# yifita/DSS

Hardware: AMD Instinct MI355X
Metric: Msplats/s fwd+bwd @512^2 (higher is better)
Workload: dtype f32; 1 GPU; BASELINE configs[1]: bunny-8000 x4 jitter = 32684 pts/cloud, 1 camera(s), 512x512, K=5, fwd+bwd (setup+raster+blend and their backward), grad_out=randn(seed 1), variance scale h precomputed (kNN-7 outside the step; see value_with_knn); points_per_cloud=32684, cameras=1, image_size=512, points_per_pixel=5, h_precomputed=True, parallelism=rows1, launch=eager, steps_per_graph_launch=1, full=False

## Files before the change

dss_amd/_lib.py:

```python
import ctypes
import os
import threading

import torch

_HERE = os.path.dirname(os.path.abspath(__file__))
LIB_PATH = os.environ.get("DSS_HIP_LIBRARY") or os.path.join(_HERE, "csrc", "libdss_hip.so")

_lib = None
_lock = threading.Lock()

_c_int, _c_i64, _c_f32, _c_vp, _c_sz = (ctypes.c_int, ctypes.c_int64, ctypes.c_float,
                                         ctypes.c_void_p, ctypes.c_size_t)

SIGNATURES = {
    "dss_version": (_c_int, []),
    "dss_last_error": (ctypes.c_char_p, []),
    "dss_band_rows": (_c_int, [_c_int, _c_int, _c_int]),
    "dss_set_option": (_c_int, [_c_int, _c_int]),
    "dss_get_option": (_c_int, [_c_int]),
    "dss_splat_forward_workspace": (_c_sz, [_c_int, _c_i64, _c_int, _c_int, _c_int]),
    "dss_splat_forward_clean_bytes": (_c_sz, [_c_int, _c_i64, _c_int]),
    "dss_splat_forward": (_c_int, [_c_vp] * 6 + [_c_int, _c_i64, _c_f32, _c_int, _c_int, _c_int, _c_int, _c_int]
                          + [_c_vp] * 5 + [_c_vp, _c_sz, _c_vp]),
# ... 77 lines not shown
    "dss_camera_backward": (_c_int, [_c_vp] * 5 + [_c_int, _c_i64, _c_int, _c_vp, _c_vp, _c_f32, _c_vp, _c_vp, _c_vp, _c_sz, _c_vp]),
    "dss_phong_backward_camera": (_c_int, [_c_vp] * 6 + [_c_int, _c_i64, _c_int] + [_c_vp] * 4 + [_c_int, _c_int, _c_vp, _c_f32,
                                                                                                 _c_vp, _c_vp, _c_sz, _c_vp]),
    "dss_phong_backward_lights_workspace": (_c_sz, [_c_int, _c_i64, _c_int]),
    "dss_phong_backward_lights": (_c_int, [_c_vp] * 6 + [_c_int, _c_i64, _c_int] + [_c_vp] * 4 + [_c_int, _c_int, _c_vp, _c_f32]
                                  + [_c_vp] * 4 + [_c_vp, _c_sz, _c_vp]),
    "dss_blend_backward": (_c_int, [_c_vp] * 10 + [_c_int, _c_i64, _c_int, _c_int, _c_int, _c_int, _c_int, _c_vp, _c_vp]),
    "dss_blend_backward_scatter": (_c_int, [_c_vp] * 4 + [_c_int] * 5 + [_c_i64, _c_vp, _c_vp]),
}


def load():
    global _lib
    if _lib is not None:
        return _lib
    with _lock:
        if _lib is None:
            if not os.path.exists(LIB_PATH):
                raise RuntimeError(
                    "dss_amd: %s not found. Build it with `make -C dss_amd/csrc` (or "
                    "`python -c 'import __graft_entry__ as g; g.build()'`). There is no CPU fallback."
                    % LIB_PATH)
            lib = ctypes.CDLL(LIB_PATH)
            for name, (res, args) in SIGNATURES.items():
                fn = getattr(lib, name)
                fn.restype = res
                fn.argtypes = args
            _lib = lib
    return _lib


WS_ORDER_SAVE, WS_ORDER_REUSE = 0x10, 0x20
WS_BAND_OUTPUTS = 0x40
OPT_LEAN_WORKSPACE, OPT_BACKWARD_TPW, OPT_BACKWARD_ADDR64, OPT_BACKWARD_FUSED, OPT_KNN_QUERY = 0, 1, 2, 3, 4


def set_option(option: int, value: int) -> int:
    lib = load()
    old = lib.dss_get_option(option)
    check(lib.dss_set_option(option, value), "dss_set_option")
    return old


def check(rc: int, what: str) -> None:
    if rc != 0:
        msg = load().dss_last_error().decode("utf-8", "replace")
        raise RuntimeError("%s failed (%d): %s" % (what, rc, msg))


def ptr(t):
    return None if t is None else ctypes.c_void_p(t.data_ptr())


def stream_ptr(device):
    return ctypes.c_void_p(torch.cuda.current_stream(device).cuda_stream)


def require_gpu(t: torch.Tensor, name: str, dtype=None) -> torch.Tensor:
    if not isinstance(t, torch.Tensor):
        raise TypeError("%s must be a torch.Tensor" % name)
    if not t.is_cuda:
        raise RuntimeError("dss_amd: %s is on %s; the HIP path needs GPU tensors (no CPU fallback)"
                           % (name, t.device))
    if dtype is not None and t.dtype != dtype:
        raise RuntimeError("dss_amd: %s must be %s, got %s" % (name, dtype, t.dtype))
    return t.contiguous()

# ... 50 lines not shown
```

dss_amd/csrc/api.hip:

```cpp
#include <stdarg.h>
#include <atomic>
#include "common.h"

namespace dss {

static thread_local char g_err[512] = "";

void set_error(const char *fmt, ...)
{
    va_list ap;
    va_start(ap, fmt);
    vsnprintf(g_err, sizeof(g_err), fmt, ap);
    va_end(ap);
}

int check_launch(const char *what)
{
    const hipError_t e = hipGetLastError();
    if (e != hipSuccess) {
        set_error("%s: %s", what, hipGetErrorString(e));
        return DSS_ERR_LAUNCH;
    }
    return DSS_OK;
}
// ... 21 lines not shown
    }
    return cus;
}

unsigned resident_blocks(int dev, const void *kernel, int block)
{
    DeviceCache *dc = (dev >= 0 && dev < DSS_MAX_DEVICES) ? &g_dev[dev] : nullptr;
    int i = 0;
    for (; dc && i < DSS_MAX_RESIDENT; ++i) {
        const void *k = dc->kernel[i].load(std::memory_order_acquire);
        if (k == nullptr) break;
        const unsigned long long v = dc->value[i].load(std::memory_order_acquire);
        if (k == kernel && (v >> 32) == (unsigned)block) return (unsigned)v;
    }
    int per_cu = 0;
    (void)hipOccupancyMaxActiveBlocksPerMultiprocessor(&per_cu, kernel, block, 0);
    (void)hipGetLastError();
    if (per_cu < 1) per_cu = 1;
    const void *expect = nullptr;
    if (dc && i < DSS_MAX_RESIDENT && dc->kernel[i].compare_exchange_strong(expect, kernel, std::memory_order_acq_rel))
        dc->value[i].store((unsigned long long)block << 32 | (unsigned)per_cu, std::memory_order_release);
    return (unsigned)per_cu;
}

}

extern "C" int dss_set_option(int option, int value)
{
    if (option < 0 || option >= DSS_OPT_COUNT) { dss::set_error("dss_set_option: unknown option %d", option); return DSS_ERR_INVALID_ARGUMENT; }
    if (option == DSS_OPT_BACKWARD_TPW && !(value == 0 || value == 1 || value == 2 || value == 4)) {
        dss::set_error("dss_set_option: DSS_OPT_BACKWARD_TPW takes 0 (automatic), 1, 2 or 4");
        return DSS_ERR_INVALID_ARGUMENT;
    }
    dss::g_opt[option].store(value, std::memory_order_relaxed);
    return DSS_OK;
}
extern "C" int dss_get_option(int option) { return dss::option(option); }

extern "C" int dss_band_rows(int row0, int row1, int row_cycle)
{
    if (row1 <= row0) return 0;
    if (row_cycle <= 1) return row1 - row0;
    const int span = row1 - row0, period = 8 * row_cycle;
    const int full = span / period, rem = span - full * period;
    return full * 8 + (rem < 8 ? rem : 8);
}

extern "C" int dss_version(void) { return DSS_HIP_VERSION; }
extern "C" const char *dss_last_error(void) { return dss::g_err; }
```

dss_amd/csrc/raster_backward.hip:

```cpp
#include <stdlib.h>
#include <type_traits>
#include "point_bodies.h"

namespace dss {

__device__ __forceinline__ uint32_t float_key(float f)
{
    const uint32_t b = __float_as_uint(f);
    return (b & 0x80000000u) ? ~b : (b | 0x80000000u);
}
__device__ __forceinline__ float key_float(uint32_t k)
{
    const uint32_t b = (k & 0x80000000u) ? (k & 0x7fffffffu) : ~k;
    return __uint_as_float(b);
}

#define MED_THREADS 256
#define MED_BINS 2048
#define MED_PTS_PER_WG 2048

__device__ __forceinline__ void select_bin(const uint32_t *hist, uint32_t k, bool k_is_lower_median,
                                           uint32_t *s_scan , uint32_t &bin_out, uint32_t &k_out,
                                           uint32_t &total_out)
{
// ... 885 lines not shown
{
    v = row_sum16(v);
    if (RP == 1) return v;
    const float a = __int_as_float(__builtin_amdgcn_readlane(__float_as_int(v), 0));
    const float b = __int_as_float(__builtin_amdgcn_readlane(__float_as_int(v), 16));
    const float c = __int_as_float(__builtin_amdgcn_readlane(__float_as_int(v), 32));
    const float d = __int_as_float(__builtin_amdgcn_readlane(__float_as_int(v), 48));
    if (RP == 4) return (a + b) + (c + d);
    return grp == 0 ? a + b : c + d;
}
template <int TPW>
__device__ __forceinline__ int tasks_max(int v)
{
    int m = __builtin_amdgcn_readlane(v, 0);
    if (TPW >= 2) m = max(m, __builtin_amdgcn_readlane(v, 32));
    if (TPW >= 4) m = max(m, max(__builtin_amdgcn_readlane(v, 16), __builtin_amdgcn_readlane(v, 48)));
    return m;
}


extern "C" __device__ unsigned long long dss_dispatch_id(void) __asm("llvm.amdgcn.dispatch.id");

#define DSS_BACKWARD_FUSED_DEFAULT 4
#define FB_THREADS 256
#define FB_BUCKETS 256
#define FB_CAND_MAX 4096
#define FB_HIST 1024
#define FB_TAG_RS 0
#define FB_TAGS (8 * 64)
#define FB_SPIN_LIMIT (1 << 20)
#define FB_ALPHA_PER_WG 2048
#define FB_MAX_SEG 256
#define FB_MEDIAN_LDS (FB_CAND_MAX + FB_HIST + 3 * FB_MAX_SEG + 32)
#define FB_KEY_LO 0xB7800000u
#define FB_KEY_HI 0xBF800000u
__device__ __forceinline__ uint32_t fb_bucket(uint32_t key)
{
    const uint32_t c = min(max(key, FB_KEY_LO), FB_KEY_HI - 1u);
    return (c - FB_KEY_LO) >> 19;
}

struct FusedPrep {
    const uint8_t *visible;
    uint32_t *seg_count;
    int32_t *vis_list;
    uint32_t *keys;
    uint32_t *chunk_hist;
    uint2 *seg_range;
    unsigned long long *tags;
    float *rs;
    int64_t P;
    int chunks, per;
    float radii_s;
};

__device__ __forceinline__ unsigned long long fb_launch_tag()
{
    const unsigned long long q = (unsigned long long)__builtin_amdgcn_queue_ptr();
    return dss_dispatch_id() * 0x9E3779B97F4A7C15ull ^ (q << 17) ^ (q >> 7) ^ 0x5851F42D4C957F2Dull;
}

__device__ __forceinline__ uint32_t fb_block_excl_scan(uint32_t v, uint32_t *s_w , uint32_t &total)
{
    const int lane = threadIdx.x & 63, wid = threadIdx.x >> 6;
    const uint32_t x = wave_incl_scan(v);
    __syncthreads();
    if (lane == 63) s_w[wid] = x;
    __syncthreads();
    uint32_t woff = 0;
    total = 0;
#pragma unroll
    for (int w = 0; w < FB_THREADS / 64; ++w) {
        const uint32_t c = s_w[w];
        if (w < wid) woff += c;
        total += c;
    }
    return woff + x - v;
}

template <int PER>
__device__ __forceinline__ void fb_prep_segment(const FusedPrep &F, int c, const float *__restrict__ radii,
                                                const int64_t *__restrict__ first_idx, const int64_t *__restrict__ num_pts,
// ... 297 lines not shown
            if (__ballot(!ok) == 0ull) break;
            __builtin_amdgcn_s_sleep(8);
        }
    }
    __syncthreads();
}

template <int PER>
__global__ __launch_bounds__(FB_THREADS) void fb_prep_kernel(const FusedPrep F, const float *__restrict__ radii,
                                                             const int64_t *__restrict__ first_idx,
                                                             const int64_t *__restrict__ num_pts, int N,
                                                             float *__restrict__ grad_pts, float *__restrict__ grad_feat, int C,
                                                             const float *__restrict__ grad_out, float *__restrict__ alpha_plane,
                                                             size_t npix)
{
    if ((int)blockIdx.x >= F.chunks) {
        const size_t i0 = (size_t)(blockIdx.x - F.chunks) * FB_ALPHA_PER_WG + threadIdx.x;
        if (C == 3) {
            const float4 *g4 = reinterpret_cast<const float4 *>(grad_out);
            float a[FB_ALPHA_PER_WG / FB_THREADS];
#pragma unroll
            for (int u = 0; u < FB_ALPHA_PER_WG / FB_THREADS; ++u) a[u] = g4[min(i0 + (size_t)u * FB_THREADS, npix - 1)].w;
#pragma unroll
            for (int u = 0; u < FB_ALPHA_PER_WG / FB_THREADS; ++u)
                if (i0 + (size_t)u * FB_THREADS < npix) alpha_plane[i0 + (size_t)u * FB_THREADS] = a[u];
        } else {
            for (int u = 0; u < FB_ALPHA_PER_WG / FB_THREADS; ++u) {
                const size_t i = i0 + (size_t)u * FB_THREADS;
                if (i < npix) alpha_plane[i] = grad_out[i * (C + 1) + C];
            }
        }
        return;
    }
    __shared__ uint32_t s_fb[2 * FB_BUCKETS + 160];
    fb_prep_segment<PER>(F, (int)blockIdx.x, radii, first_idx, num_pts, N, grad_pts, grad_feat, C, s_fb);
}
__global__ __launch_bounds__(FB_THREADS) void fb_median_kernel(const FusedPrep F, const int64_t *__restrict__ first_idx,
                                                               const int64_t *__restrict__ num_pts)
{
    __shared__ uint32_t s_fb[FB_MEDIAN_LDS];
    const float v = fb_median(F, (int)blockIdx.x, first_idx, num_pts, s_fb);
    if (threadIdx.x == 0) F.rs[blockIdx.x] = v;
}

#ifndef DSS_BAND_RB
#define DSS_BAND_RB 8
#endif
#define BAND_SHARE 512
template <int C, bool SEG, int TPW, bool A32, bool CYC = false, bool PREP = false, bool BAND = false>
__global__ __launch_bounds__(256) void render_backward_kernel(
    const float *__restrict__ grad_out, const float *__restrict__ grad_alpha ,
    const int32_t *__restrict__ idx, const float *__restrict__ qv,
    const float *__restrict__ wsum, const float *__restrict__ scaler, const float *__restrict__ points,
    const float *__restrict__ radii, const float *__restrict__ rs, const int64_t *__restrict__ first_idx,
    const int64_t *__restrict__ num_pts, const uint32_t *__restrict__ vis_count,
    const int32_t *__restrict__ vis_list, int n_seg, int seg_pts, int N, int S, int K, int Crt, float clip, int row0,
    int rows, uint32_t large_waves, float *__restrict__ grad_feat, float *__restrict__ grad_pts, int tshift = 3,
    const float *__restrict__ world = nullptr ,
    const float *__restrict__ Mproj = nullptr ,
    const FusedPrep F = FusedPrep() ,
    int astride = 1 ,
    const OwnArgs OW = OwnArgs{nullptr, 1} )
{
    constexpr int CM = (C > 0) ? C : BLEND_MAX_C;
    constexpr int KF = 8;
    constexpr int GS = 64 / TPW;
// ... 53 lines not shown
        return chunked ? ((t / max(CH, 1u)) * 8u + xcd) * CH + (t % max(CH, 1u)) : t;
    };
    const uint32_t wave_u = (uint32_t)__builtin_amdgcn_readfirstlane((int)qof(t0));
    if (!PREP && !BAND && wave_u >= n_groups) return;
    const bool has_tasks = wave < n_waves && wave_u < n_groups;
    const uint32_t t_first = (uint32_t)__builtin_amdgcn_readfirstlane((int)t0);

    auto task_ids = [&](uint32_t q) -> int {
        int off[TPW];
#pragma unroll
        for (int g = 0; g < TPW; ++g) {
            const uint32_t t = (uint32_t)TPW * q + (uint32_t)g;
            off[g] = -1;
            if (t < count) {
                if (SEG) {
                    const int seg = (int)__popcll(__ballot(seg_excl <= t)) - 1;
                    const uint32_t excl = (uint32_t)__builtin_amdgcn_readlane((int)seg_excl, seg);
                    off[g] = seg * seg_pts + (int)(t - excl);
                } else {
                    off[g] = (int)t;
                }
            }
        }
        int o = off[0];
#pragma unroll
        for (int g = 1; g < TPW; ++g) o = (grp == g) ? off[g] : o;
        return o >= 0 ? vis_list[o] : -1;
    };
    const NdcMap ndc(S);
    const size_t plane = (size_t)rows * S;
    __shared__ uint32_t s_deal[2];
    const uint32_t blk4 = (blockIdx.x - first_block) * 4u;
    auto dyn_group = [&](uint32_t i) -> uint32_t { return blk4 + (i & 3u) + (i >> 2) * n_waves; };
    float *s_rec = reinterpret_cast<float *>(s_pool);
    int32_t *s_band = reinterpret_cast<int32_t *>(s_pool) + (BAND ? 7 * BAND_SHARE : 0);
    __shared__ uint32_t s_bcnt[2];
    __shared__ float s_brs[BAND ? 64 : 1];
    constexpr int BAND_NSH = 24;
    int32_t b_id[2] = {-1, -1};
    int b_n[2] = {-1, -1};
    float b_py[2] = {0.f, 0.f}, b_ry[2] = {0.f, 0.f};
    if (BAND) {
        if (threadIdx.x == 0) { s_bcnt[0] = 0; s_bcnt[1] = 0; }
        __syncthreads();
        const uint32_t n_wg = gridDim.x - first_block, wg = blockIdx.x - first_block;
#pragma unroll
        for (int j = 0; j < 2; ++j) {
            const uint32_t e = wg + ((uint32_t)threadIdx.x + 256u * (uint32_t)j) * n_wg;
            if (e < count) {
                int sg = 0;
#pragma unroll
                for (int st = FB_MAX_SEG / 2; st >= 1; st >>= 1) sg += (sg + st < FB_MAX_SEG && s_bseg[sg + st] <= e) ? st : 0;
                b_id[j] = vis_list[(size_t)sg * seg_pts + (e - s_bseg[sg])];
            }
        }
#pragma unroll
        for (int j = 0; j < 2; ++j) {
            if (b_id[j] >= 0) {
                const size_t i = (size_t)b_id[j];
                const int slot = (int)threadIdx.x + 256 * j;
                const float px_ = points[3 * i], py_ = points[3 * i + 1], pz_ = points[3 * i + 2];
                const float2 rr_ = reinterpret_cast<const float2 *>(radii)[i];
                const float sc_ = scaler ? scaler[i] : 0.0f;
                b_py[j] = py_;
                b_ry[j] = rr_.y;
                b_n[j] = find_cloud(b_id[j], first_idx, num_pts, N);
// ... 29 lines not shown
                }
            }
            const unsigned long long m = __ballot(keep);
            uint32_t base = 0;
            if (lane == 0 && m) base = atomicAdd(&s_bcnt[WHICH], (uint32_t)__popcll(m));
            base = (uint32_t)__builtin_amdgcn_readfirstlane((int)base);
            if (keep) {
                s_band[WHICH * BAND_SHARE + base + __builtin_amdgcn_mbcnt_hi((unsigned)(m >> 32), __builtin_amdgcn_mbcnt_lo((unsigned)m, 0u))] =
                    (int)threadIdx.x + 256 * j;
            } else if (b_id[j] >= 0) {
                const size_t i = (size_t)b_id[j];
                if (WHICH == 0) {
                    if (grad_feat)
                        for (int ch = 0; ch < Cn; ++ch) grad_feat[i * Cn + ch] = 0.0f;
                } else {
                    grad_pts[3 * i] = 0.0f; grad_pts[3 * i + 1] = 0.0f; grad_pts[3 * i + 2] = 0.0f;
                }
            }
        }
        __syncthreads();
    };
    const uint32_t wave_in_wg = threadIdx.x >> 6;
    auto band_ids = [&](uint32_t q, int which) -> int {
        const uint32_t t = (uint32_t)TPW * q + (uint32_t)grp;
        return t < s_bcnt[which] ? s_band[which * BAND_SHARE + t] : -1;
    };
    if (PREP || BAND) {
        if (threadIdx.x < 2) s_deal[threadIdx.x] = 4u;
        __syncthreads();
    }
    auto run_tasks = [&](auto phase_tag) {
    constexpr int PH = decltype(phase_tag)::value;
    uint32_t t_cur = t_first;
    const uint32_t b_groups = BAND ? (s_bcnt[PH == 2 ? 1 : 0] + TPW - 1u) / TPW : 0u;
    int p_nx = BAND ? band_ids(wave_in_wg, PH == 2 ? 1 : 0) : task_ids(wave_u);
    for (;;) {
        const int b_slot = BAND ? max(p_nx, 0) : 0;
        const int b_word = (BAND && p_nx >= 0) ? reinterpret_cast<const int32_t *>(s_rec)[b_slot] : -1;
        const int p = BAND ? (b_word >= 0 ? (b_word & ((1 << BAND_NSH) - 1)) : -1) : p_nx;
        const int p_cloud = b_word >= 0 ? (b_word >> BAND_NSH) : -1;
        uint32_t t_next, q_next;
        if (BAND) {
            uint32_t i_next = 0;
            if (lane == 0) i_next = atomicAdd(&s_deal[PH == 2 ? 1 : 0], 1u);
            q_next = t_next = (uint32_t)__builtin_amdgcn_readfirstlane((int)i_next);
        } else if (PREP) {
            uint32_t i_next = 0;
            if (lane == 0) i_next = atomicAdd(&s_deal[PH == 2 ? 1 : 0], 1u);
            q_next = t_next = dyn_group((uint32_t)__builtin_amdgcn_readfirstlane((int)i_next));
        } else {
            t_next = t_cur + t_stride;
            q_next = qof(t_next);
        }
        const bool more = q_next < (BAND ? b_groups : n_groups);
        if (more) p_nx = BAND ? band_ids(q_next, PH == 2 ? 1 : 0) : task_ids(q_next);
        float px = 0.f, py = 0.f, pz = -1.f, rx = 0.f, ry = 0.f, sc = 0.f, cur_r = 0.f;
        float wx = 0.f, wy = 0.f, wz = 0.f;
        int n = -1;
        if (BAND) {
            if (p >= 0) {
                px = s_rec[BAND_SHARE + b_slot]; py = s_rec[2 * BAND_SHARE + b_slot]; pz = s_rec[3 * BAND_SHARE + b_slot];
                rx = s_rec[4 * BAND_SHARE + b_slot]; ry = s_rec[5 * BAND_SHARE + b_slot]; sc = s_rec[6 * BAND_SHARE + b_slot];
                n = p_cloud;
                if (PH != 1) cur_r = s_brs[n];
            }
        } else if (p >= 0) {
            px = points[3 * (size_t)p]; py = points[3 * (size_t)p + 1]; pz = points[3 * (size_t)p + 2];
            const float2 rr = reinterpret_cast<const float2 *>(radii)[p];
            rx = rr.x; ry = rr.y;
            sc = scaler ? scaler[p] : 0.0f;
            if (world) { wx = world[3 * (size_t)p]; wy = world[3 * (size_t)p + 1]; wz = world[3 * (size_t)p + 2]; }
            for (int cld = 0; cld < N; ++cld) {
                const int64_t f = first_idx[cld];
                const bool own = (int64_t)p >= f && (int64_t)p < f + num_pts[cld];
                n = own ? cld : n;
                if (PH != 1) cur_r = own ? (PREP ? __hip_atomic_load(&rs[cld], __ATOMIC_RELAXED, __HIP_MEMORY_SCOPE_AGENT) : rs[cld]) : cur_r;
            }
        }
        const int nn = max(n, 0);
        typedef float f2 __attribute__((ext_vector_type(2)));
        f2 gx2 = {0.0f, 0.0f}, gy2 = {0.0f, 0.0f};
        if constexpr (PH != 1) {
// ... 227 lines not shown
#pragma unroll
                    for (int k = 0; k < KF; ++k) {
                        vi[k] = -1; qk[k] = 0.0f;
                        if (k < K) { vi[k] = pi[k]; qk[k] = pq[k]; }
                    }
                    cum = wsum[pix];
#pragma unroll
                    for (int ch = 0; ch < CM; ++ch) gch[ch] = (ch < Cn) ? go[ch] : 0.0f;
#pragma unroll
                    for (int k = 0; k < KF; ++k) {
                        const bool hit = (k < K) && vi[k] == (int32_t)p;
                        q_sel = hit ? qk[k] : q_sel;
                        found = found || hit;
                    }
                } else {
                    cum = 0.0f;
                    for (int k = 0; k < K; ++k) {
                        const int32_t v = pi[k];
                        if (v == (int32_t)p) { found = true; q_sel = pq[k]; }
                        if (!wsum && v >= 0) cum += ewa_weight(pq[k], scaler[v]);
                    }
                    if (wsum) cum = wsum[pix];
                    else if (cum < 1e-4f) cum = 1e-4f;
#pragma unroll
                    for (int ch = 0; ch < CM; ++ch) gch[ch] = (ch < Cn) ? go[ch] : 0.0f;
                }
                if (!found) continue;
                const float wn = ewa_weight(q_sel, sc) * fast_rcp(cum);
#pragma unroll
                for (int ch = 0; ch < CM; ++ch)
                    if (ch < Cn) acc[ch] = fmaf(gch[ch], wn, acc[ch]);
            }
        }
        if (PH != 1) {
            gx = task_sum<RP>(gx, grp);
            gy = task_sum<RP>(gy, grp);
        }
        if (PH != 2) {
#pragma unroll
            for (int ch = 0; ch < CM; ++ch)
                if (ch < Cn) acc[ch] = task_sum<RP>(acc[ch], grp);
        }
        if (PH == 1) {
            if (l == 0 && rp == 0 && p >= 0 && n >= 0 && grad_feat) {
#pragma unroll
                for (int ch = 0; ch < CM; ++ch)
                    if (ch < Cn) grad_feat[(size_t)p * Cn + ch] = acc[ch];
            }
        } else if (l == 0 && rp == 0 && p >= 0 && n >= 0) {
            if (clip > 0.0f) {
                const float nrm = sqrtf(gx * gx + gy * gy);
                const float k = fminf(nrm, clip) * fast_rcp(fmaxf(nrm, 1e-12f));
                gx *= k;
                gy *= k;
            }
            float o0 = gx, o1 = gy, o2 = 0.0f;
            if (world) {
                const float *m = Mproj + 16 * nn;
                const float cx = wx * m[0] + wy * m[4] + wz * m[8] + m[12];
                const float cy = wx * m[1] + wy * m[5] + wz * m[9] + m[13];
                const float w = wx * m[3] + wy * m[7] + wz * m[11] + m[15];
                const float iw = 1.0f / w;
                const float nx = cx * iw, ny = cy * iw;
                float t3[3];
#pragma unroll
                for (int i = 0; i < 3; ++i) {
                    const float jx = (m[i * 4 + 0] - nx * m[i * 4 + 3]) * iw;
                    const float jy = (m[i * 4 + 1] - ny * m[i * 4 + 3]) * iw;
                    t3[i] = jx * gx + jy * gy + 0.0f;
                }
                o0 = t3[0]; o1 = t3[1]; o2 = t3[2];
            }
            grad_pts[3 * (size_t)p] = o0;
            grad_pts[3 * (size_t)p + 1] = o1;
            grad_pts[3 * (size_t)p + 2] = o2;
            if (PH == 0 && grad_feat) {
#pragma unroll
                for (int ch = 0; ch < CM; ++ch)
                    if (ch < Cn) grad_feat[(size_t)p * Cn + ch] = acc[ch];
            }
        }
        if (!more) break;
        t_cur = t_next;
    }
    };
    if (BAND) {
        PREP_MARK(0);
        if (grad_feat) {
            band_filter(std::integral_constant<int, 0>{});
            PREP_MARK(8);
            if (wave_in_wg * TPW < s_bcnt[0]) run_tasks(std::integral_constant<int, 1>{});
        }
        PREP_MARK(1);
        if (PREP) fb_wait_rs(F, N, fb_launch_tag());
        if ((int)threadIdx.x < N)
            s_brs[threadIdx.x] = PREP ? __hip_atomic_load(&rs[threadIdx.x], __ATOMIC_RELAXED, __HIP_MEMORY_SCOPE_AGENT) : rs[threadIdx.x];
        __syncthreads();
        PREP_MARK(2);
        band_filter(std::integral_constant<int, 1>{});
        PREP_MARK(9);
        if (wave_in_wg * TPW < s_bcnt[1]) run_tasks(std::integral_constant<int, 2>{});
        PREP_MARK(3);
    } else if (!PREP) {
        run_tasks(std::integral_constant<int, 0>{});
    } else {
        PREP_MARK(0);
        if (has_tasks) run_tasks(std::integral_constant<int, 1>{});
        PREP_MARK(1);
        fb_wait_rs(F, N, fb_launch_tag());
        PREP_MARK(2);
        if (has_tasks) run_tasks(std::integral_constant<int, 2>{});
        PREP_MARK(3);
    }
// ... 2 lines not shown
__global__ __launch_bounds__(256) void zbuf_backward_kernel(const int32_t *__restrict__ idx,
                                                            const float *__restrict__ grad_zbuf,
                                                            size_t npix, int K, float *__restrict__ grad_pts)
{
    const size_t i = (size_t)blockIdx.x * blockDim.x + threadIdx.x;
    if (i >= npix) return;
    for (int k = 0; k < K; ++k) {
        const float g = grad_zbuf[i * K + k];
        if (g == 0.0f) continue;
        const int32_t p = idx[i * K + k];
        if (p < 0) break;
        atomicAdd(&grad_pts[3 * (size_t)p + 2], g);
    }
}

__global__ __launch_bounds__(256) void clip_grad_kernel(float *__restrict__ grad, int64_t P, float clip)
{
    const int64_t p = (int64_t)blockIdx.x * blockDim.x + threadIdx.x;
    if (p >= P) return;
    const float gx = grad[3 * p], gy = grad[3 * p + 1], gz = grad[3 * p + 2];
    const float nrm = sqrtf(gx * gx + gy * gy + gz * gz);
    const float scaler = fminf(nrm, clip);
    const float den = fmaxf(nrm, 1e-12f);
    grad[3 * p] = gx / den * scaler;
    grad[3 * p + 1] = gy / den * scaler;
    grad[3 * p + 2] = gz / den * scaler;
}

}

using namespace dss;

struct PrepLayout {
    size_t seg_count, vis_list, vis_keys, chunk_hist, seg_range, rs, alpha, tags, bytes;
    int chunks, per;
    int f_chunks, f_per;
};
static PrepLayout prep_layout(int N, int64_t P, int S, bool band = false)
{
    PrepLayout L;
    const size_t n = N > 0 ? N : 1, p = P > 0 ? (size_t)P : 1;
    L.per = prep_points_per_thread(P);
    const size_t seg = (size_t)L.per * PREP_THREADS;
    L.chunks = (int)((p + seg - 1) / seg);
    L.f_per = 1;
    const size_t f_max_seg = (band && p > (size_t)2 * FB_THREADS * PREP_MAX_SEG) ? FB_MAX_SEG : PREP_MAX_SEG;
    while (L.f_per < 16 && (size_t)L.f_per * FB_THREADS * f_max_seg < p) L.f_per *= 2;
    L.f_chunks = (int)((p + (size_t)L.f_per * FB_THREADS - 1) / ((size_t)L.f_per * FB_THREADS));
    size_t off = 0;
    L.seg_count = off;  off += (size_t)FB_MAX_SEG * 4;
    L.vis_list = off;   off += align_up(p * 4, 256);
    L.vis_keys = off;   off += align_up(p * 8, 256);
    L.chunk_hist = off; off += align_up(n * (size_t)FB_MAX_SEG * 256 * 4, 256);
    L.seg_range = off;  off += align_up(n * (size_t)FB_MAX_SEG * 8, 256);
    L.tags = off;       off += align_up((size_t)FB_TAGS * 8, 256);
    L.rs = off;         off += align_up(n * 4, 256);
    L.alpha = off;      off += align_up(n * (size_t)(S > 0 ? S : 0) * (size_t)(S > 0 ? S : 0) * 4, 256);
    L.bytes = off;
    return L;
}

struct LongLayout {
    size_t hist, vis_count, vis_list, rs, alpha, cell_of, sorted, cell_start, cell_total, block_hist, bytes;
};
static LongLayout long_layout(int N, int64_t P, int S)
{
    LongLayout L;
    const size_t n = N > 0 ? N : 1, s = S > 0 ? S : 1, p = P > 0 ? (size_t)P : 1;
    const size_t cells = (size_t)make_cells(N > 0 ? N : 1, S > 0 ? S : 1).total;
    size_t off = 0;
    L.hist = off;       L.vis_count = off + 3 * n * MED_BINS * 4;
    off += align_up(3 * n * MED_BINS * 4 + 256, 256);
    L.vis_list = off;   off += align_up(p * 4, 256);
    L.rs = off;         off += align_up(n * 4, 256);
    L.alpha = off;      off += align_up(n * s * s * 4, 256);
    L.cell_of = off;    off += align_up(p * 4, 256);
    L.sorted = off;     off += align_up(p * 4, 256);
    L.cell_start = off; off += align_up(cells * 4, 256);
    L.cell_total = off; off += align_up(cells * 4, 256);
    L.block_hist = off; off += align_up(cell_blocks(P) * cells * 4, 256);
    L.bytes = off;
    return L;
}

static const decltype(&backward_compact_kernel<2>) compact_by_per[] = {backward_compact_kernel<2>, backward_compact_kernel<4>};
static const decltype(&band_filter_kernel<2>) band_filter_by_per[] = {band_filter_kernel<2>, band_filter_kernel<4>};
static const decltype(&fb_prep_kernel<1>) fb_prep_by_per[] = {fb_prep_kernel<1>, fb_prep_kernel<2>, fb_prep_kernel<4>,
                                                              fb_prep_kernel<8>, fb_prep_kernel<16>};
// ... 223 lines not shown
        }
    }
    const int rows = dss_band_rows(row0, row1, row_cycle);
    int tshift = 3;
    for (int c = row_cycle; c > 1; c >>= 1) ++tshift;
    const bool cyc = row_cycle > 1;
    if (P == 0) return DSS_OK;
    if (P > 0x7ffffff0ll) { set_error("dss_render_backward: P too large"); return DSS_ERR_UNSUPPORTED; }
    OwnArgs OW = {(grad_full != nullptr && (rows < S || cyc)) ? grad_full + C : nullptr, C + 1};
    const bool own_given = occ_full != nullptr && (rows < S || cyc);
    if (own_given) { OW.alpha = occ_full; OW.astride = 1; }
    const int own = OW.alpha != nullptr ? 1 : 0;
    if (!grad_out || !points || !radii || !visible || !first_idx || !num_pts || !grad_pts ||
        (grad_feat && (!idx || !qvalue || !scaler))) {
        set_error("dss_render_backward: NULL tensor pointer");
        return DSS_ERR_INVALID_ARGUMENT;
    }
    const size_t need = dss_render_backward_workspace(N, P, S);
    if (!workspace || workspace_bytes < need) {
        set_error("dss_render_backward: workspace %zu bytes < required %zu", workspace_bytes, need);
        return DSS_ERR_WORKSPACE;
    }
    if (((uintptr_t)grad_out & 15u) && C == 3) { set_error("dss_render_backward: grad_out must be 16-byte aligned"); return DSS_ERR_INVALID_ARGUMENT; }

    hipStream_t st = as_stream(stream);
    char *w = reinterpret_cast<char *>(workspace);
    const bool small = P <= PREP_MAX_POINTS;
    const size_t npix = (size_t)N * rows * S;
    int dev = 0;
    (void)hipGetDevice(&dev);
    const int n_cus = cu_count(dev);
    const unsigned cap = (unsigned)n_cus * resident_blocks(dev, (const void *)gather_kernel({C == 3, true, 4, true, false, false, false}), 256);
    const unsigned pgrid = (unsigned)((P + 3) / 4 < cap ? (P + 3) / 4 : cap);
    auto gather_grid = [&](const GatherVariant &v, bool fused_launch) -> unsigned {
        if (fused_launch && !v.prep) return pgrid;
        const unsigned g = std::min(pgrid, (unsigned)n_cus * resident_blocks(dev, (const void *)gather_kernel(v), 256));
        return v.prep ? std::max(g, (unsigned)N + 8u) : g;
    };
    const uint32_t large_waves = 6u * (uint32_t)n_cus * 4u;
    const int tpw_opt = option(DSS_OPT_BACKWARD_TPW);
    const long long est_tasks = (long long)P * 2 / 5;
    int tpw = est_tasks >= 16ll * cap * 4 ? 4 : (est_tasks >= 4ll * cap * 4 ? 2 : 1);
    if (tpw_opt == 1 || tpw_opt == 2 || tpw_opt == 4) tpw = tpw_opt;
    unsigned long long widest = (unsigned long long)N * (unsigned long long)rows * (unsigned long long)S *
                                (unsigned long long)(K > C + 1 ? K : C + 1) * 4ull;
    if (own) widest = std::max(widest, (unsigned long long)N * (unsigned long long)S * (unsigned long long)S * (unsigned long long)(own_given ? 1 : C + 1) * 4ull);
    const bool a32 = widest < (1ull << 32) && option(DSS_OPT_BACKWARD_ADDR64) != 1;
    if (!a32) tpw = 4;
    if (!a32 && world) { set_error("dss_render_backward: the fused projection needs gathered tensors below 4 GB"); return DSS_ERR_UNSUPPORTED; }
    int fused_opt = option(DSS_OPT_BACKWARD_FUSED);
    if (fused_opt == 0) fused_opt = DSS_BACKWARD_FUSED_DEFAULT;
    const bool band = rows < S || cyc;
    bool fused = small && (fused_opt == 4 || fused_opt == 5) && a32 && N <= 64 && (unsigned)N + 8u <= pgrid &&
                 (!band || (fused_opt == 4 && (!cyc || C == 3) && world == nullptr));
    if (fused && fused_opt == 4 && !(tpw_opt == 1 || tpw_opt == 2 || tpw_opt == 4)) {
        const long long est = band ? est_tasks * 2 * rows / S : est_tasks;
        tpw = est >= 16ll * cap * 4 ? 4 : (est >= 1ll * cap * 4 ? 2 : 1);
        if (cyc) tpw = 4;
    }
    GatherVariant v = {C == 3, small, tpw, a32, cyc, fused && (band || (run_prep && fused_opt != 5)), fused && band};
    if (v.band && (long long)BAND_SHARE * ((long long)gather_grid(v, true) - N) < (long long)P) fused = v.prep = v.band = false;

    int n_seg = 0, seg_pts = 0;
    uint32_t *vis_count;
    int32_t *vis_list;
    float *rs;
    const float *alpha;
    FusedPrep FP = FusedPrep();
    if (fused) {
        const PrepLayout L = prep_layout(N, P, S, band);
        n_seg = L.f_chunks;
        seg_pts = L.f_per * FB_THREADS;
        vis_count = reinterpret_cast<uint32_t *>(w + L.seg_count);
        vis_list = reinterpret_cast<int32_t *>(w + L.vis_list);
        rs = rs_out ? rs_out : reinterpret_cast<float *>(w + L.rs);
        FP.visible = visible; FP.seg_count = vis_count; FP.vis_list = vis_list;
        FP.keys = reinterpret_cast<uint32_t *>(w + L.vis_keys);
        FP.chunk_hist = reinterpret_cast<uint32_t *>(w + L.chunk_hist);
        FP.seg_range = reinterpret_cast<uint2 *>(w + L.seg_range);
        FP.tags = reinterpret_cast<unsigned long long *>(w + L.tags);
        FP.rs = rs; FP.P = P;
        FP.chunks = L.f_chunks; FP.per = L.f_per; FP.radii_s = radii_s;
        float *plane = reinterpret_cast<float *>(w + L.alpha);
        alpha = plane;
        const float *plane_src = own ? grad_full : grad_out;
        const size_t plane_px = own_given ? (size_t)0 : (own ? (size_t)N * S * S : npix);
        if (own && !own_given) { OW.alpha = plane; OW.astride = 1; }
        if (run_prep) {
            const unsigned alpha_wgs = (unsigned)((plane_px + FB_ALPHA_PER_WG - 1) / FB_ALPHA_PER_WG);
            hipLaunchKernelGGL(fb_prep_by_per[__builtin_ctz(L.f_per)], dim3((unsigned)L.f_chunks + alpha_wgs), dim3(FB_THREADS), 0,
                               st, FP, radii, first_idx, num_pts, N, grad_pts, grad_feat, C, plane_src, plane, plane_px);
            if (fused_opt == 5)
                hipLaunchKernelGGL(fb_median_kernel, dim3((unsigned)N), dim3(FB_THREADS), 0, st, FP, first_idx, num_pts);
        }
    } else if (small) {
        const PrepLayout L = prep_layout(N, P, S);
        n_seg = L.chunks;
        seg_pts = L.per * PREP_THREADS;
        alpha = reinterpret_cast<const float *>(w + L.alpha);
        vis_count = reinterpret_cast<uint32_t *>(w + L.seg_count);
        vis_list = reinterpret_cast<int32_t *>(w + L.vis_list);
        rs = rs_out ? rs_out : reinterpret_cast<float *>(w + L.rs);
        if (run_prep)
            launch_prep(radii, visible, first_idx, num_pts, N, P, radii_s, rs, w, L, grad_pts, grad_feat, C, grad_out, npix, st);
        if (run_prep && rows < S)
            hipLaunchKernelGGL(band_filter_by_per[L.per == 2 ? 0 : 1], dim3(L.chunks), dim3(PREP_THREADS), 0, st, points, radii,
                               rs, first_idx, num_pts, N, S, row0, rows, vis_count, vis_list, grad_pts, grad_feat, C, tshift, own);
    } else {
        const LongLayout L = long_layout(N, P, S);
        const CellGrid cg = make_cells(N, S);
        uint32_t *hist = reinterpret_cast<uint32_t *>(w + L.hist);
        vis_count = reinterpret_cast<uint32_t *>(w + L.vis_count);
        int32_t *unsorted = reinterpret_cast<int32_t *>(w + L.vis_list);
// ... 105 lines not shown
```

include/dss_hip.h:

```cpp
#ifndef DSS_HIP_H
#define DSS_HIP_H

#include <stddef.h>
#include <stdint.h>

#ifdef __cplusplus
extern "C" {
#endif

#define DSS_HIP_VERSION 103

#if defined(__GNUC__)
#define DSS_API __attribute__((visibility("default")))
#else
#define DSS_API
#endif

#define DSS_OK 0
#define DSS_ERR_INVALID_ARGUMENT (-1)
#define DSS_ERR_WORKSPACE (-2)
#define DSS_ERR_UNSUPPORTED (-3)
#define DSS_ERR_LAUNCH (-4)

#define DSS_MAX_K_FAST 32
#define DSS_MAX_K 150

DSS_API int dss_version(void);
DSS_API const char *dss_last_error(void);

#define DSS_OPT_LEAN_WORKSPACE 0
#define DSS_OPT_BACKWARD_TPW 1
#define DSS_OPT_BACKWARD_ADDR64 2
#define DSS_OPT_BACKWARD_FUSED 3
#define DSS_OPT_KNN_QUERY 4
#define DSS_OPT_COUNT 5
DSS_API int dss_band_rows(int row0, int row1, int row_cycle);
DSS_API int dss_set_option(int option, int value);
DSS_API int dss_get_option(int option);

DSS_API size_t dss_splat_forward_workspace(int N, int64_t P, int S, int K, int bin_size);
DSS_API size_t dss_splat_forward_clean_bytes(int N, int64_t P, int S);

DSS_API int dss_splat_forward(const float *points, const float *ellipse, const float *cutoff,
                      const float *radii, const int64_t *first_idx, const int64_t *num_pts,
                      int N, int64_t P, float merge_thr, int S, int K, int bin_size,
                      int row0, int row1,
                      int32_t *idx, float *zbuf, float *qvalue, float *occ, uint8_t *visible,
                      void *workspace, size_t workspace_bytes, void *stream);

DSS_API int dss_splat_bin(const float *points, const float *radii, const int64_t *first_idx,
                          const int64_t *num_pts, int N, int64_t P, int S, int row0, int row1,
                          void *workspace, size_t workspace_bytes, void *stream);
DSS_API int dss_splat_fine(const float *points, const float *ellipse, const float *cutoff,
                           const float *radii, const int64_t *first_idx, const int64_t *num_pts,
                           int N, int64_t P, float merge_thr, int S, int K, int row0, int row1,
                           int32_t *idx, float *zbuf, float *qvalue, float *occ, uint8_t *visible,
                           const void *workspace, size_t workspace_bytes, void *stream);

DSS_API int dss_splat_fine_blend(const float *points, const float *ellipse, const float *cutoff,
                                 const float *radii, const int64_t *first_idx, const int64_t *num_pts,
                                 int N, int64_t P, float merge_thr, int S, int K, int row0, int row1,
                                 int32_t *idx, float *zbuf, float *qvalue, float *occ, uint8_t *visible,
                                 const float *scaler, const float *feat, int C, float *image, float *wsum,
                                 const void *workspace, size_t workspace_bytes, void *stream);


DSS_API size_t dss_backward_radius_workspace(int N, int64_t P);
DSS_API int dss_backward_radius(const float *radii, const uint8_t *visible, const int64_t *first_idx,
// ... 278 lines not shown
```

Before: 567.0 Msplats/s.

## Add global claim counters for tail groups in fused backward gather

In the prep-fused, non-band backward gather, waves that exhaust the per-workgroup static deal of full rounds switch to claiming leftover task groups from 128 cache-line-padded global atomic counters, which the prep kernel zeroes. The intent is to balance the ragged tail of phase-2 work across waves instead of leaving it to fixed assignment. It also adds a DSS_OPT_BACKWARD_GRID option to cap the gather grid size, defaulting to off. The cost is extra global atomics and a dependency on the prep kernel having reset the counters.

```diff
diff --git a/dss_amd/_lib.py b/dss_amd/_lib.py
--- a/dss_amd/_lib.py
+++ b/dss_amd/_lib.py
@@ -133,7 +133,7 @@
 
 WS_ORDER_SAVE, WS_ORDER_REUSE = 0x10, 0x20
 WS_BAND_OUTPUTS = 0x40
-OPT_LEAN_WORKSPACE, OPT_BACKWARD_TPW, OPT_BACKWARD_ADDR64, OPT_BACKWARD_FUSED, OPT_KNN_QUERY = 0, 1, 2, 3, 4
+OPT_LEAN_WORKSPACE, OPT_BACKWARD_TPW, OPT_BACKWARD_ADDR64, OPT_BACKWARD_FUSED, OPT_KNN_QUERY, OPT_BACKWARD_GRID = 0, 1, 2, 3, 4, 5
 
 
 def set_option(option: int, value: int) -> int:
diff --git a/dss_amd/csrc/api.hip b/dss_amd/csrc/api.hip
--- a/dss_amd/csrc/api.hip
+++ b/dss_amd/csrc/api.hip
@@ -77,6 +77,10 @@
         dss::set_error("dss_set_option: DSS_OPT_BACKWARD_TPW takes 0 (automatic), 1, 2 or 4");
         return DSS_ERR_INVALID_ARGUMENT;
     }
+    if (option == DSS_OPT_BACKWARD_GRID && value < 0) {
+        dss::set_error("dss_set_option: DSS_OPT_BACKWARD_GRID takes 0 (automatic) or a positive number of workgroups");
+        return DSS_ERR_INVALID_ARGUMENT;
+    }
     dss::g_opt[option].store(value, std::memory_order_relaxed);
     return DSS_OK;
 }
diff --git a/dss_amd/csrc/raster_backward.hip b/dss_amd/csrc/raster_backward.hip
--- a/dss_amd/csrc/raster_backward.hip
+++ b/dss_amd/csrc/raster_backward.hip
@@ -941,6 +941,9 @@
 #define FB_ALPHA_PER_WG 2048
 #define FB_MAX_SEG 256
 #define FB_MEDIAN_LDS (FB_CAND_MAX + FB_HIST + 3 * FB_MAX_SEG + 32)
+#define FB_CLAIM_CTRS 128
+#define FB_CLAIM_LINE 32
+#define FB_CLAIM_WORDS (FB_CLAIM_CTRS * FB_CLAIM_LINE)
 #define FB_KEY_LO 0xB7800000u
 #define FB_KEY_HI 0xBF800000u
 __device__ __forceinline__ uint32_t fb_bucket(uint32_t key)
@@ -957,6 +960,7 @@
     uint32_t *chunk_hist;
     uint2 *seg_range;
     unsigned long long *tags;
+    uint32_t *claim;
     float *rs;
     int64_t P;
     int chunks, per;
@@ -1320,6 +1324,7 @@
         }
         return;
     }
+    if (blockIdx.x == 0 && F.claim != nullptr && threadIdx.x < FB_CLAIM_CTRS) F.claim[(size_t)threadIdx.x * FB_CLAIM_LINE] = 0u;
     __shared__ uint32_t s_fb[2 * FB_BUCKETS + 160];
     fb_prep_segment<PER>(F, (int)blockIdx.x, radii, first_idx, num_pts, N, grad_pts, grad_feat, C, s_fb);
 }
@@ -1439,6 +1444,11 @@
     __shared__ uint32_t s_deal[2];
     const uint32_t blk4 = (blockIdx.x - first_block) * 4u;
     auto dyn_group = [&](uint32_t i) -> uint32_t { return blk4 + (i & 3u) + (i >> 2) * n_waves; };
+    constexpr bool CLAIM = PREP && !BAND;
+    const uint32_t full_rounds = n_groups / max(n_waves, 1u);
+    const uint32_t claim_base = full_rounds * n_waves;
+    const bool claimable = CLAIM && full_rounds >= 1u && claim_base < n_groups;
+    const uint32_t claim_slot = (uint32_t)__builtin_amdgcn_readfirstlane((int)(wave & (FB_CLAIM_CTRS - 1u)));
     float *s_rec = reinterpret_cast<float *>(s_pool);
     int32_t *s_band = reinterpret_cast<int32_t *>(s_pool) + (BAND ? 7 * BAND_SHARE : 0);
     __shared__ uint32_t s_bcnt[2];
@@ -1534,6 +1544,9 @@
     auto run_tasks = [&](auto phase_tag) {
     constexpr int PH = decltype(phase_tag)::value;
     uint32_t t_cur = t_first;
+    constexpr bool CL = CLAIM && PH == 2;
+    uint32_t *claim_ctr = CL ? F.claim + (size_t)claim_slot * FB_CLAIM_LINE : nullptr;
+    bool claiming = false;
     const uint32_t b_groups = BAND ? (s_bcnt[PH == 2 ? 1 : 0] + TPW - 1u) / TPW : 0u;
     int p_nx = BAND ? band_ids(wave_in_wg, PH == 2 ? 1 : 0) : task_ids(wave_u);
     for (;;) {
@@ -1547,9 +1560,14 @@
             if (lane == 0) i_next = atomicAdd(&s_deal[PH == 2 ? 1 : 0], 1u);
             q_next = t_next = (uint32_t)__builtin_amdgcn_readfirstlane((int)i_next);
         } else if (PREP) {
-            uint32_t i_next = 0;
-            if (lane == 0) i_next = atomicAdd(&s_deal[PH == 2 ? 1 : 0], 1u);
-            q_next = t_next = dyn_group((uint32_t)__builtin_amdgcn_readfirstlane((int)i_next));
+            q_next = t_next = 0xffffffffu;
+            if (!(CL && claiming)) {
+                uint32_t i_next = 0;
+                if (lane == 0) i_next = atomicAdd(&s_deal[PH == 2 ? 1 : 0], 1u);
+                i_next = (uint32_t)__builtin_amdgcn_readfirstlane((int)i_next);
+                if (CL && claimable && i_next >= 4u * full_rounds) claiming = true;
+                else q_next = t_next = dyn_group(i_next);
+            }
         } else {
             t_next = t_cur + t_stride;
             q_next = qof(t_next);
@@ -1843,6 +1861,9 @@
                     if (ch < Cn) acc[ch] = fmaf(gch[ch], wn, acc[ch]);
             }
         }
+        uint32_t ticket = 0;
+        if (CL && claiming && lane == 0)
+            ticket = __hip_atomic_fetch_add(claim_ctr, 1u, __ATOMIC_RELAXED, __HIP_MEMORY_SCOPE_AGENT);
         if (PH != 1) {
             gx = task_sum<RP>(gx, grp);
             gy = task_sum<RP>(gy, grp);
@@ -1890,6 +1911,13 @@
                 for (int ch = 0; ch < CM; ++ch)
                     if (ch < Cn) grad_feat[(size_t)p * Cn + ch] = acc[ch];
             }
+        }
+        if (CL && claiming) {
+            const uint32_t q_claim = claim_base + claim_slot +
+                                     (uint32_t)__builtin_amdgcn_readfirstlane((int)ticket) * FB_CLAIM_CTRS;
+            if (q_claim >= n_groups) break;
+            p_nx = task_ids(q_claim);
+            continue;
         }
         if (!more) break;
         t_cur = t_next;
@@ -1958,7 +1986,7 @@
 using namespace dss;
 
 struct PrepLayout {
-    size_t seg_count, vis_list, vis_keys, chunk_hist, seg_range, rs, alpha, tags, bytes;
+    size_t seg_count, vis_list, vis_keys, chunk_hist, seg_range, rs, alpha, tags, claim, bytes;
     int chunks, per;
     int f_chunks, f_per;
 };
@@ -1980,6 +2008,7 @@
     L.chunk_hist = off; off += align_up(n * (size_t)FB_MAX_SEG * 256 * 4, 256);
     L.seg_range = off;  off += align_up(n * (size_t)FB_MAX_SEG * 8, 256);
     L.tags = off;       off += align_up((size_t)FB_TAGS * 8, 256);
+    L.claim = off;      off += align_up((size_t)FB_CLAIM_WORDS * 4, 256);
     L.rs = off;         off += align_up(n * 4, 256);
     L.alpha = off;      off += align_up(n * (size_t)(S > 0 ? S : 0) * (size_t)(S > 0 ? S : 0) * 4, 256);
     L.bytes = off;
@@ -2269,10 +2298,13 @@
     const int n_cus = cu_count(dev);
     const unsigned cap = (unsigned)n_cus * resident_blocks(dev, (const void *)gather_kernel({C == 3, true, 4, true, false, false, false}), 256);
     const unsigned pgrid = (unsigned)((P + 3) / 4 < cap ? (P + 3) / 4 : cap);
+    const int grid_opt = option(DSS_OPT_BACKWARD_GRID);
     auto gather_grid = [&](const GatherVariant &v, bool fused_launch) -> unsigned {
-        if (fused_launch && !v.prep) return pgrid;
-        const unsigned g = std::min(pgrid, (unsigned)n_cus * resident_blocks(dev, (const void *)gather_kernel(v), 256));
-        return v.prep ? std::max(g, (unsigned)N + 8u) : g;
+        if (fused_launch && !v.prep) return grid_opt > 0 ? std::min(pgrid, std::max((unsigned)grid_opt, (unsigned)N + 8u)) : pgrid;
+        unsigned g = std::min(pgrid, (unsigned)n_cus * resident_blocks(dev, (const void *)gather_kernel(v), 256));
+        if (v.prep) g = std::max(g, (unsigned)N + 8u);
+        if (grid_opt > 0) g = std::min(g, std::max((unsigned)grid_opt, (unsigned)N + 8u));
+        return g;
     };
     const uint32_t large_waves = 6u * (uint32_t)n_cus * 4u;
     const int tpw_opt = option(DSS_OPT_BACKWARD_TPW);
@@ -2316,6 +2348,7 @@
         FP.chunk_hist = reinterpret_cast<uint32_t *>(w + L.chunk_hist);
         FP.seg_range = reinterpret_cast<uint2 *>(w + L.seg_range);
         FP.tags = reinterpret_cast<unsigned long long *>(w + L.tags);
+        FP.claim = reinterpret_cast<uint32_t *>(w + L.claim);
         FP.rs = rs; FP.P = P;
         FP.chunks = L.f_chunks; FP.per = L.f_per; FP.radii_s = radii_s;
         float *plane = reinterpret_cast<float *>(w + L.alpha);
diff --git a/include/dss_hip.h b/include/dss_hip.h
--- a/include/dss_hip.h
+++ b/include/dss_hip.h
@@ -33,7 +33,8 @@
 #define DSS_OPT_BACKWARD_ADDR64 2
 #define DSS_OPT_BACKWARD_FUSED 3
 #define DSS_OPT_KNN_QUERY 4
-#define DSS_OPT_COUNT 5
+#define DSS_OPT_BACKWARD_GRID 5
+#define DSS_OPT_COUNT 6
 DSS_API int dss_band_rows(int row0, int row1, int row_cycle);
 DSS_API int dss_set_option(int option, int value);
 DSS_API int dss_get_option(int option);
```

Measured after the change: 578.5 Msplats/s (median of 6 runs). +2.0%, better.
